# cmeraki/audiotoken

Measured on AMD Instinct MI355X. Metric: audio-sec tokenized / wall-sec (acoustic + semantic_m), higher is better.
Workload: dtype f32 (linear layers: two fp16 pieces per operand, three MFMA products, fp32 accumulate)

## Files before the change

audiotoken_amd/csrc/attention_f16x2_w8.hip:

```cpp
#include "at_common.h"
#include "w2vbert_kernels.h"
#include "split_scheme.h"

#include <cstdio>
#include <type_traits>

namespace at {

typedef __attribute__((address_space(3))) void w8_lds_void;

#ifdef W8_DEBUG_STAMPS
__device__ unsigned long long w8_stamps[2][12];
#define W8_T(i) const unsigned long long w8_t##i = __builtin_readcyclecounter()
#define W8_ACC(k, a_, b_) w8_d[k] += w8_t##b_ - w8_t##a_
#else
#define W8_T(i) do {} while (0)
#define W8_ACC(k, a_, b_) do {} while (0)
#endif

constexpr int W8_QB = 256, W8_KB = 64;
constexpr int W8_PLANE_B = W8_KB * 64 * 2;
constexpr int W8_TILE_B = 2 * W8_PLANE_B;
constexpr int W8_KBUFS = 2, W8_VBUFS = 2;
constexpr int W8_KV_B = (W8_KBUFS + W8_VBUFS) * W8_TILE_B;
constexpr int W8_QE_LD = 73;
constexpr int W8_LDS_MAX = 163840;
constexpr float W8_SCALE2 = 0.125f * 1.4426950408889634f;
constexpr float W8_P_LOG2 = 10.0f;
constexpr float W8_DEFER = 4.0f;
#ifndef W8_P_PIECES
#define W8_P_PIECES 2
#endif
constexpr int W8_PP = W8_P_PIECES;

static size_t w8_lds_bytes(int T, bool relpos) {
    const int nkt = (T + W8_KB - 1) / W8_KB;
    return (size_t)W8_KV_B + (relpos ? (size_t)W8_QB * W8_QE_LD * 4 : 0) + (size_t)nkt * W8_KB * 4 + 16;
}

__device__ __forceinline__ float w8_pair_max(float x) {
    const auto r = __builtin_amdgcn_permlane32_swap(__float_as_uint(x), __float_as_uint(x), false, false);
    return fmaxf(__uint_as_float(r[0]), __uint_as_float(r[1]));
}
__device__ __forceinline__ float w8_pair_sum(float x) {
    const auto r = __builtin_amdgcn_permlane32_swap(__float_as_uint(x), __float_as_uint(x), false, false);
    return __uint_as_float(r[0]) + __uint_as_float(r[1]);
}

__device__ __forceinline__ void w8_split_pair(float p0, float p1, unsigned& hi, unsigned& lo) {
    asm("v_cvt_pk_f16_f32 %0, %1, %2" : "=v"(hi) : "v"(p0), "v"(p1));
    asm("v_fma_mixlo_f16 %0, -%1, 1.0, %2 op_sel:[0,0,0] op_sel_hi:[1,0,0]" : "=v"(lo) : "v"(hi), "v"(p0));
    asm("v_fma_mixhi_f16 %0, -%1, 1.0, %2 op_sel:[1,0,0] op_sel_hi:[1,0,0]" : "+v"(lo) : "v"(hi), "v"(p1));
}

constexpr int W8_NQB = 1;
template <bool RELPOS>
__global__ __launch_bounds__(512 / W8_NQB, W8_NQB == 1 ? 2 : 1) void relpos_attention_w8_kernel(const float* __restrict__ qkv, const float* __restrict__ amask,
                                                                     const _Float16* __restrict__ dist_pieces, float dist_inv_scale, float* __restrict__ ctx, int T, int hid,
                                                                     int* __restrict__ status, _Float16* __restrict__ ctx_pieces, long long rows_pad,
                                                                     int nheads, int nclips, const _Float16* __restrict__ kv_pieces) {
    constexpr int NQB = W8_NQB;
    typedef SchemeF16x2 SC;
    typedef _Float16 PT;
    typedef f16x8 V8;
    typedef f16x4 V4;
    constexpr float XS = XB_F16_ACT_SCALE;
    constexpr float S_SCALE2 = W8_SCALE2 / (XS * XS);
    RangeMax over;
    extern __shared__ __attribute__((aligned(16))) unsigned char smem_raw[];
    const int nkt = (T + W8_KB - 1) / W8_KB;
    unsigned char* KV = smem_raw;
    float* QE = reinterpret_cast<float*>(KV + W8_KV_B);
    float* kbt = QE + (RELPOS ? W8_QB * W8_QE_LD : 0);
    int* tmask = reinterpret_cast<int*>(kbt + nkt * W8_KB);
    const int tid = threadIdx.x, lane = tid & 63;
    constexpr int NW = 8 / NQB, QW = 32 * NQB, NT = 64 * NW;
    const int wave = __builtin_amdgcn_readfirstlane(tid >> 6);
    const int l32 = lane & 31, hh = lane >> 5;
    const int nqt = (T + W8_QB - 1) / W8_QB;
    const int nblk = gridDim.x, per_xcd = (nblk + 7) >> 3;
    const int lid = (int)(blockIdx.x & 7) * per_xcd + (int)(blockIdx.x >> 3);
    if (lid >= nqt * nheads * nclips) return;
    const int qt = lid % nqt, pair = lid / nqt;
    const int h = pair % nheads, b = pair / nheads;
    const int l0 = qt * W8_QB;
    const long long rowbase = (long long)b * T;
    const int LD = 3 * hid;
    const float* qp = qkv + h * 64;

    const unsigned plane_b = (unsigned)(rows_pad * (long long)hid * 2);
    const __amdgpu_buffer_rsrc_t kvrs = __builtin_amdgcn_make_buffer_rsrc((void*)kv_pieces, 0, (int)(4u * plane_b), 0x00020000);
    constexpr int RW = 8 * NQB;
    const int d_row = wave * RW + (lane >> 3), d_cs = lane & 7;
    const unsigned clip_b = (unsigned)(rowbase * hid * 2 + h * 128);
    const int row_b = hid * 2;
    auto issue_k = [&](int kt, int buf) {
#pragma unroll
        for (int j = 0; j < NQB; ++j) {
            const int row = min(kt * W8_KB + d_row + 8 * j, T - 1);
            const unsigned vo = clip_b + (unsigned)(row * row_b) + ((d_cs ^ (((d_row + 8 * j) >> 1) & 7)) << 4);
#pragma unroll
            for (int p = 0; p < 2; ++p)
                __builtin_amdgcn_raw_ptr_buffer_load_lds(kvrs, (w8_lds_void*)(KV + buf * W8_TILE_B + wave * (RW * 128) + p * W8_PLANE_B + j * 1024), 16, vo, p * plane_b, 0, 0);
        }
    };
    auto issue_v = [&](int kt, int buf) {
#pragma unroll
        for (int j = 0; j < NQB; ++j) {
            const int row = min(kt * W8_KB + d_row + 8 * j, T - 1);
            const unsigned vo = clip_b + (unsigned)(row * row_b) + ((d_cs ^ ((((d_row + 8 * j) >> 1) & 1) << 2)) << 4);
#pragma unroll
            for (int p = 0; p < 2; ++p)
                __builtin_amdgcn_raw_ptr_buffer_load_lds(kvrs, (w8_lds_void*)(KV + (W8_KBUFS + buf) * W8_TILE_B + wave * (RW * 128) + p * W8_PLANE_B + j * 1024), 16, vo,
                                                         (2u + p) * plane_b, 0, 0);
        }
    };
    issue_k(0, 0);
    issue_v(0, 0);
    if (nkt > 1) issue_k(1, 1);

    const float FMIN = -3.4028234663852886e38f;
    if (tid < 2) tmask[tid] = 0;
    __syncthreads();
    for (int k = tid; k < nkt * W8_KB; k += NT) {
        float v = -INFINITY;
        if (k < T) v = amask[rowbase + k] != 0.f ? 0.f : FMIN;
        kbt[k] = v;
        if (v != 0.f) atomicOr(&tmask[k >> 11], 1 << ((k >> 6) & 31));
    }
    const int lq0 = l0 + wave * QW + l32;
    V8 qpc[NQB][2][4];
#pragma unroll
    for (int qb = 0; qb < NQB; ++qb) {
        const int lq = lq0 + 32 * qb;
        const int lc = lq < T ? lq : T - 1;
#pragma unroll
        for (int ds = 0; ds < 4; ++ds) {
            const f4 a = *reinterpret_cast<const f4*>(qp + (rowbase + lc) * LD + ds * 16 + 8 * hh);
            const f4 c = *reinterpret_cast<const f4*>(qp + (rowbase + lc) * LD + ds * 16 + 8 * hh + 4);
            V4 pa[2], pc[2];
            over |= split4<SC>(a, XS, pa);
            over |= split4<SC>(c, XS, pc);
#pragma unroll
            for (int i = 0; i < 2; ++i)
#pragma unroll
                for (int k = 0; k < 4; ++k) { qpc[qb][i][ds][k] = pa[i][k]; qpc[qb][i][ds][4 + k] = pc[i][k]; }
        }
    }
    if constexpr (RELPOS) {
        const float qe_scale = W8_SCALE2 * dist_inv_scale / XS;
#pragma unroll
        for (int qb = 0; qb < NQB; ++qb) {
            float* row = QE + (wave * QW + qb * 32 + l32) * W8_QE_LD;
#pragma unroll
            for (int rt = 0; rt < 3; ++rt) {
                f16v acc;
#pragma unroll
                for (int r = 0; r < 16; ++r) acc[r] = 0.f;
#pragma unroll
                for (int ds = 0; ds < 4; ++ds) {
                    V8 ef[2];
#pragma unroll
                    for (int p = 0; p < 2; ++p) ef[p] = *reinterpret_cast<const V8*>(dist_pieces + (p * 96 + rt * 32 + l32) * 64 + ds * 16 + 8 * hh);
#pragma unroll
                    for (int t = 0; t < SC::NPROD; ++t) acc = SC::mfma(ef[SC::prod_a(t)], qpc[qb][SC::prod_w(t)][ds], acc);
                }
#pragma unroll
                for (int r = 0; r < 16; ++r) {
                    const int bucket = rt * 32 + 8 * (r >> 2) + 4 * hh + (r & 3);
                    if (bucket < W8_QE_LD) row[bucket] = qe_scale * acc[r];
                }
            }
        }
    }
    f16v oacc[NQB][2];
#pragma unroll
    for (int qb = 0; qb < NQB; ++qb)
#pragma unroll
        for (int dt = 0; dt < 2; ++dt)
#pragma unroll
            for (int r = 0; r < 16; ++r) oacc[qb][dt][r] = 0.f;
    float mrun[NQB], lrun[NQB], alpha[NQB];
    bool rescale[NQB];
#pragma unroll
    for (int qb = 0; qb < NQB; ++qb) { mrun[qb] = -INFINITY; lrun[qb] = 0.f; alpha[qb] = 0.f; }
    const int wl_min = l0 + wave * QW, wl_max = wl_min + QW - 1;
    int koff[4];
#pragma unroll
    for (int ds = 0; ds < 4; ++ds) koff[ds] = l32 * 128 + (((2 * ds + hh) ^ ((l32 >> 1) & 7)) << 4);
    int voff[2];
    {
        const int li = lane & 15, vq = li >> 2, vp = li & 3;
        const int c0 = ((lane & 16) >> 3) + (vp >> 1), sv = (vq >> 1) & 1;
#pragma unroll
        for (int dt = 0; dt < 2; ++dt) voff[dt] = (4 * hh + vq) * 128 + ((((dt ^ sv) << 2) + c0) << 4) + (vp & 1) * 8;
    }
    asm volatile("s_waitcnt vmcnt(0)" ::: "memory");
    __syncthreads();
    const int tm0 = __builtin_amdgcn_readfirstlane(tmask[0]), tm1 = __builtin_amdgcn_readfirstlane(tmask[1]);
    typedef const __attribute__((address_space(3))) float lds_cf;
    typedef const __attribute__((address_space(3))) f4 lds_cf4;
    lds_cf* qe0 = (lds_cf*)(QE + (wave * QW + l32) * W8_QE_LD);
    lds_cf* kbt3 = (lds_cf*)kbt;
    float c_left[NQB], c_right[NQB];
#pragma unroll
    for (int qb = 0; qb < NQB; ++qb) { c_left[qb] = 0.f; c_right[qb] = 0.f; }
    if constexpr (RELPOS) {
#pragma unroll
        for (int qb = 0; qb < NQB; ++qb) { c_left[qb] = qe0[qb * 32 * W8_QE_LD]; c_right[qb] = qe0[qb * 32 * W8_QE_LD + 72]; }
    }

    auto s_tile = [&](f16v (&s)[NQB][2], int kbuf) {
        const unsigned char* Kb = KV + kbuf * W8_TILE_B;
#pragma unroll
        for (int kh = 0; kh < 2; ++kh) {
#pragma unroll
            for (int qb = 0; qb < NQB; ++qb)
#pragma unroll
                for (int r = 0; r < 16; ++r) s[qb][kh][r] = 0.f;
#pragma unroll
            for (int ds = 0; ds < 4; ++ds) {
                V8 kf[2];
#pragma unroll
                for (int p = 0; p < 2; ++p) kf[p] = *reinterpret_cast<const V8*>(Kb + p * W8_PLANE_B + kh * 32 * 128 + koff[ds]);
#pragma unroll
                for (int t = 0; t < SC::NPROD; ++t)
#pragma unroll
                    for (int qb = 0; qb < NQB; ++qb) s[qb][kh] = SC::mfma(kf[SC::prod_a(t)], qpc[qb][SC::prod_w(t)][ds], s[qb][kh]);
            }
        }
    };
    auto tile_fast = [&](int kt, bool& far_left) -> bool {
        const int r0 = kt * W8_KB;
        far_left = (r0 + W8_KB - 1) - wl_min <= -64;
        const bool far_right = r0 - wl_max >= 8;
        const bool masked = (((kt < 32 ? tm0 : tm1) >> (kt & 31)) & 1) != 0;
        return (!RELPOS || far_left || far_right) && !masked;
    };
    auto bias_pass = [&](f16v (&s)[2], int r0, int lq, lds_cf* qe, float c_far, auto near_) -> float {
        constexpr bool NEAR = decltype(near_)::value;
        float mx = -INFINITY;
#pragma unroll
        for (int kh = 0; kh < 2; ++kh)
#pragma unroll
            for (int g = 0; g < 4; ++g) {
                const int key0 = kh * 32 + 8 * g + 4 * hh;
                const f4 kb4 = *(lds_cf4*)(kbt3 + r0 + key0);
#pragma unroll
                for (int e = 0; e < 4; ++e) {
                    float bias = c_far;
                    if constexpr (NEAR) {
                        int dd = (r0 + key0 + e) - lq;
                        dd = dd < -64 ? -64 : (dd > 8 ? 8 : dd);
                        bias = qe[dd + 64];
                    }
                    const float sc = fmaf(S_SCALE2, s[kh][4 * g + e], bias + kb4[e]);
                    s[kh][4 * g + e] = sc;
                    mx = fmaxf(mx, sc);
                }
            }
        return mx;
    };
    auto softmax_general = [&](f16v (&s)[2], int kt, int qb) {
        const int r0 = kt * W8_KB;
        const int bmin = wl_min + 32 * qb, bmax = bmin + 31;
        const bool far_left = (r0 + W8_KB - 1) - bmin <= -64;
        const bool far_right = r0 - bmax >= 8;
        float mx;
        if (!RELPOS || far_left || far_right) mx = bias_pass(s, r0, 0, qe0, far_left ? c_left[qb] : c_right[qb], std::false_type{});
        else mx = bias_pass(s, r0, lq0 + 32 * qb, qe0 + qb * 32 * W8_QE_LD, 0.f, std::true_type{});
        mx = w8_pair_max(mx);
        const bool resc = __builtin_amdgcn_ballot_w64(mx > mrun[qb] + W8_DEFER) != 0ull;
        rescale[qb] = resc;
        const float mnew = resc ? fmaxf(mrun[qb], mx) : mrun[qb];
        const float sub = mnew - W8_P_LOG2;
        float rs = 0.f;
#pragma unroll
        for (int kh = 0; kh < 2; ++kh)
#pragma unroll
            for (int r = 0; r < 16; ++r) {
                const float p = __builtin_amdgcn_exp2f(s[kh][r] - sub);
                s[kh][r] = p;
                rs += p;
            }
        rs = w8_pair_sum(rs);
        alpha[qb] = resc ? __builtin_amdgcn_exp2f(mrun[qb] - mnew) : 1.0f;
        lrun[qb] = lrun[qb] * alpha[qb] + rs;
        mrun[qb] = mnew;
    };
    float f_mraw[NQB], f_mnew[NQB], f_bias2[NQB], f_rs[NQB], f_cfar[NQB];
    auto stat_slice = [&](f16v (&sa)[2], int qb, int k) {
        if (k < 4) {
            if (k == 0) { f_mraw[qb] = -INFINITY; f_rs[qb] = 0.f; }
#pragma unroll
            for (int e = 0; e < 8; ++e) f_mraw[qb] = fmaxf(f_mraw[qb], sa[k >> 1][8 * (k & 1) + e]);
        } else if (k == 4) {
            const float mx = w8_pair_max(fmaf(S_SCALE2, f_mraw[qb], f_cfar[qb]));
            const bool resc = __builtin_amdgcn_ballot_w64(mx > mrun[qb] + W8_DEFER) != 0ull;
            rescale[qb] = resc;
            f_mnew[qb] = resc ? fmaxf(mrun[qb], mx) : mrun[qb];
            f_bias2[qb] = (f_cfar[qb] - f_mnew[qb]) + W8_P_LOG2;
            alpha[qb] = resc ? __builtin_amdgcn_exp2f(mrun[qb] - f_mnew[qb]) : 1.0f;
        } else if (k < 21) {
#pragma unroll
            for (int e = 0; e < 2; ++e) {
                const int r = 2 * (k - 5) + e;
                const float p = __builtin_amdgcn_exp2f(fmaf(S_SCALE2, sa[r >> 4][r & 15], f_bias2[qb]));
                sa[r >> 4][r & 15] = p;
                f_rs[qb] += p;
            }
        } else if (k == 21) {
            const float rs = w8_pair_sum(f_rs[qb]);
            lrun[qb] = lrun[qb] * alpha[qb] + rs;
            mrun[qb] = f_mnew[qb];
        }
    };
    auto s_tile_softmax = [&](f16v (&sb)[NQB][2], int kbuf, f16v (&sa)[NQB][2]) {
        const unsigned char* Kb = KV + kbuf * W8_TILE_B;
        V8 kf[3][2];
        auto load_k = [&](int g) {
#pragma unroll
            for (int p = 0; p < 2; ++p) kf[g % 3][p] = *reinterpret_cast<const V8*>(Kb + p * W8_PLANE_B + (g >> 2) * 32 * 128 + koff[g & 3]);
        };
        load_k(0);
        load_k(1);
#pragma unroll
        for (int qb = 0; qb < NQB; ++qb)
#pragma unroll
            for (int kh = 0; kh < 2; ++kh)
#pragma unroll
                for (int r = 0; r < 16; ++r) sb[qb][kh][r] = 0.f;
        __builtin_amdgcn_sched_barrier(0);
#pragma unroll
        for (int g = 0; g < 8; ++g) {
            if (g + 2 < 8) load_k(g + 2);
#pragma unroll
            for (int t = 0; t < SC::NPROD; ++t)
#pragma unroll
                for (int qb = 0; qb < NQB; ++qb) {
                    sb[qb][g >> 2] = SC::mfma(kf[g % 3][SC::prod_a(t)], qpc[qb][SC::prod_w(t)][g & 3], sb[qb][g >> 2]);
                    const int sl = (3 * g + t) * NQB + qb;
                    if (sl < 22) stat_slice(sa[0], 0, sl);
                    else if (NQB > 1 && sl < 44) stat_slice(sa[NQB - 1], NQB - 1, sl - 22);
                    __builtin_amdgcn_sched_barrier(0);
                }
        }
    };
    auto pv_split = [&](const f16v (&s)[NQB][2], int vbuf) {
        const unsigned char* Vb = KV + (W8_KBUFS + vbuf) * W8_TILE_B;
        typedef short s4_ __attribute__((__vector_size__(4 * sizeof(short))));
        typedef unsigned u4_ __attribute__((ext_vector_type(4)));
        u4_ pp[2][NQB][2];
        auto split_pair = [&](int ks, int qb, int j) {
            unsigned hi, lo;
            if constexpr (W8_PP == 2) {
                w8_split_pair(s[qb][ks >> 1][8 * (ks & 1) + j], s[qb][ks >> 1][8 * (ks & 1) + j + 1], hi, lo);
                pp[ks & 1][qb][1][j >> 1] = lo;
            } else {
                asm("v_cvt_pk_f16_f32 %0, %1, %2" : "=v"(hi) : "v"(s[qb][ks >> 1][8 * (ks & 1) + j]), "v"(s[qb][ks >> 1][8 * (ks & 1) + j + 1]));
            }
            pp[ks & 1][qb][0][j >> 1] = hi;
        };
        V8 vf[2][2];
        auto load_v = [&](int u) {
#pragma unroll
            for (int p = 0; p < 2; ++p) {
                const unsigned char* vb = Vb + p * W8_PLANE_B + (u >> 1) * 16 * 128 + voff[u & 1];
                const s4_ lo = __builtin_amdgcn_ds_read_tr16_b64_v4i16((__attribute__((address_space(3))) s4_*)(vb));
                const s4_ hi = __builtin_amdgcn_ds_read_tr16_b64_v4i16((__attribute__((address_space(3))) s4_*)(vb + 8 * 128));
#pragma unroll
                for (int k = 0; k < 4; ++k) {
                    vf[u & 1][p][k] = __builtin_bit_cast(PT, (short)lo[k]);
                    vf[u & 1][p][4 + k] = __builtin_bit_cast(PT, (short)hi[k]);
                }
            }
        };
        load_v(0);
#pragma unroll
        for (int qb = 0; qb < NQB; ++qb)
#pragma unroll
            for (int j = 0; j < 8; j += 2) split_pair(0, qb, j);
        asm volatile("s_nop 1");
        __builtin_amdgcn_sched_barrier(0);
#pragma unroll
        for (int u = 0; u < 8; ++u) {
            const int ks = u >> 1, dt = u & 1;
            if (u + 1 < 8) load_v(u + 1);
            constexpr int T0 = W8_PP == 2 ? 0 : 1;
#pragma unroll
            for (int t = T0; t < SC::NPROD; ++t)
#pragma unroll
                for (int qb = 0; qb < NQB; ++qb) {
                    oacc[qb][dt] = SC::mfma(vf[u & 1][SC::prod_a(t)], __builtin_bit_cast(V8, pp[ks & 1][qb][SC::prod_w(t)]), oacc[qb][dt]);
                    const int sl = (dt * (SC::NPROD - T0) + (t - T0)) * NQB + qb;
                    if (ks + 1 < 4 && sl < 4 * NQB) split_pair(ks + 1, sl >> 2, 2 * (sl & 3));
                    __builtin_amdgcn_sched_barrier(0);
                }
        }
    };
#ifdef W8_DEBUG_STAMPS
    unsigned long long w8_d[8] = {0, 0, 0, 0, 0, 0, 0, 0};
    const unsigned long long w8_begin = __builtin_readcyclecounter();
#endif
    auto interval = [&](int i, f16v (&sa)[NQB][2], f16v (&sb)[NQB][2]) {
        W8_T(0);
        asm volatile("s_waitcnt vmcnt(0)" ::: "memory");
        W8_T(1);
        __builtin_amdgcn_s_barrier();
        W8_T(2);
        const bool more = i + 1 < nkt;
        if (i + 2 < nkt) issue_k(i + 2, i & 1);
        if (more) issue_v(i + 1, (i + 1) & 1);
        bool far_left;
        const bool fast = tile_fast(i, far_left);
        W8_T(3);
        if (more && fast) {
#pragma unroll
            for (int qb = 0; qb < NQB; ++qb) f_cfar[qb] = far_left ? c_left[qb] : c_right[qb];
            s_tile_softmax(sb, (i + 1) & 1, sa);
        } else {
            if (more) s_tile(sb, (i + 1) & 1);
            __builtin_amdgcn_sched_barrier(0);
            if (fast) {
#pragma unroll
                for (int qb = 0; qb < NQB; ++qb) {
                    f_cfar[qb] = far_left ? c_left[qb] : c_right[qb];
#pragma unroll
                    for (int k = 0; k < 22; ++k) stat_slice(sa[qb], qb, k);
                }
            } else {
#pragma unroll
                for (int qb = 0; qb < NQB; ++qb) softmax_general(sa[qb], i, qb);
            }
        }
        __builtin_amdgcn_sched_barrier(0);
        W8_T(4);
#pragma unroll
        for (int qb = 0; qb < NQB; ++qb)
            if (rescale[qb]) {
#pragma unroll
                for (int dt = 0; dt < 2; ++dt)
#pragma unroll
                    for (int r = 0; r < 16; ++r) oacc[qb][dt][r] *= alpha[qb];
            }
        __builtin_amdgcn_sched_barrier(0);
        W8_T(5);
        pv_split(sa, i & 1);
        W8_T(6);
#ifdef W8_DEBUG_STAMPS
        W8_ACC(0, 0, 1); W8_ACC(1, 1, 2); W8_ACC(2, 2, 3); W8_ACC(fast && more ? 3 : 4, 3, 4); W8_ACC(5, 4, 5); W8_ACC(6, 5, 6);
        w8_d[7] += (fast && more) ? 1 : 0;
#endif
    };
    f16v sA[NQB][2], sB[NQB][2];
    s_tile(sA, 0);
    for (int i = 0; i < nkt; i += 2) {
        interval(i, sA, sB);
        if (i + 1 < nkt) interval(i + 1, sB, sA);
    }
#ifdef W8_DEBUG_STAMPS
    if (blockIdx.x == (gridDim.x / 2) + 8 && (threadIdx.x == 0 || threadIdx.x == NT / 2)) {
        const int g = threadIdx.x ? 1 : 0;
        for (int k = 0; k < 8; ++k) w8_stamps[g][k] = w8_d[k];
        w8_stamps[g][8] = __builtin_readcyclecounter() - w8_begin;
        w8_stamps[g][9] = (unsigned long long)nkt;
    }
#endif
#pragma unroll
    for (int qb = 0; qb < NQB; ++qb) {
        const int lq = lq0 + 32 * qb;
        if (lq < T) {
            const float inv = (1.0f / lrun[qb]) * (1.0f / XS);
#pragma unroll
            for (int dt = 0; dt < 2; ++dt)
#pragma unroll
                for (int g = 0; g < 4; ++g) {
                    const f4 v = {oacc[qb][dt][4 * g] * inv, oacc[qb][dt][4 * g + 1] * inv, oacc[qb][dt][4 * g + 2] * inv, oacc[qb][dt][4 * g + 3] * inv};
                    if (ctx_pieces)
                        over |= store_pieces4<SC>(ctx_pieces, rows_pad * hid, rows_pad, rowbase + lq, h * 64 + dt * 32 + 8 * g + 4 * hh, v, XS);
                    else
                        *reinterpret_cast<f4*>(ctx + (rowbase + lq) * hid + h * 64 + dt * 32 + 8 * g + 4 * hh) = v;
                }
        }
    }
    range_publish(status, status ? status + 1 : nullptr, over);
}

bool relpos_attention_w8_eligible(int T, int heads, long long rows_pad, long long B, bool relpos) {
    return T >= 1 && T <= 4096  && rows_pad * heads * 64 * 8 < (1ll << 32)  && w8_lds_bytes(T, relpos) <= (size_t)W8_LDS_MAX && rows_pad >= B * T && (long long)T * heads * 64 * 2 < (1ll << 31);
}

int launch_relpos_attention_w8(const AttnArgs& a, hipStream_t stream) {
    const float *qkv = a.qkv, *amask = a.amask;
    float* const ctx = a.ctx;
    const int B = a.B, T = a.T, heads = a.heads;
    int* const status = a.status;
    __bf16* const ctx_pieces = a.ctx_pieces;
    const long long rows_pad = a.rows_pad;
    const __bf16 *kv_pieces = a.kv_pieces, *dist_pieces = a.dist.p;
    const float dist_scale = a.dist.s;
    AT_REQUIRE(kv_pieces != nullptr && relpos_attention_w8_eligible(T, heads, rows_pad, B, dist_pieces != nullptr),
               "relpos_attention_w8: needs pre-split k / v and a clip whose key-bias table fits LDS (T <= 1728 with rel-pos)");
    const long long nblk = (long long)((T + W8_QB - 1) / W8_QB) * heads * B;
    dim3 grid((unsigned)((nblk + 7) / 8 * 8));
    const size_t lds = w8_lds_bytes(T, dist_pieces != nullptr);
    const size_t lds_max = W8_LDS_MAX;
    int rc;
    const int hid = heads * 64;
    _Float16* cp = reinterpret_cast<_Float16*>(ctx_pieces);
    const _Float16* kp = reinterpret_cast<const _Float16*>(kv_pieces);
    const _Float16* dp = reinterpret_cast<const _Float16*>(dist_pieces);
    const float dinv = dist_pieces ? 1.0f / dist_scale : 1.0f;
    if (dist_pieces) {
        static LdsAttrFlags lds_attr;
        rc = set_max_dynamic_lds(lds_attr, relpos_attention_w8_kernel<true>, lds_max);
        if (!rc) hipLaunchKernelGGL((relpos_attention_w8_kernel<true>), grid, dim3(512 / W8_NQB), lds, stream, qkv, amask, dp, dinv, ctx, T, hid, status, cp, rows_pad, heads, B, kp);
    } else {
        static LdsAttrFlags lds_attr;
        rc = set_max_dynamic_lds(lds_attr, relpos_attention_w8_kernel<false>, lds_max);
        if (!rc) hipLaunchKernelGGL((relpos_attention_w8_kernel<false>), grid, dim3(512 / W8_NQB), lds, stream, qkv, amask, dp, dinv, ctx, T, hid, status, cp, rows_pad, heads, B, kp);
    }
    if (rc) return rc;
    AT_CHECK_HIP(hipGetLastError());
#ifdef W8_DEBUG_STAMPS
    {
        static int printed = 0;
        if (printed < 3) {
            ++printed;
            (void)hipStreamSynchronize(stream);
            unsigned long long hb[2][12];
            (void)hipMemcpyFromSymbol(hb, HIP_SYMBOL(w8_stamps), sizeof(hb));
            for (int g = 0; g < 2; ++g) {
                const double n = (double)(hb[g][9] ? hb[g][9] : 1), nf = (double)(hb[g][7] ? hb[g][7] : 1), ng = n - hb[g][7] > 0 ? n - hb[g][7] : 1;
                std::fprintf(stderr, "w8 stamps B %d T %d heads %d wave %d (cycles per 64-key interval, 64 queries): dma wait %.0f  barrier %.0f  issue+classify %.0f  phase A fast %.0f (x%llu)  phase A general/last %.0f (x%.0f)  rescale %.0f  phase B %.0f | loop total %.0f per interval, %llu intervals\n",
                             B, T, heads, g * 4, hb[g][0] / n, hb[g][1] / n, hb[g][2] / n, hb[g][3] / nf, hb[g][7], hb[g][4] / ng, ng, hb[g][5] / n, hb[g][6] / n, hb[g][8] / n, hb[g][9]);
            }
        }
    }
#endif
    return 0;
}

__global__ __launch_bounds__(256) void dist_split_kernel(const float* __restrict__ e, _Float16* __restrict__ out, float scale) {
    const int q = blockIdx.x * 256 + threadIdx.x;
    if (q >= 96 * 16) return;
    const int row = q >> 4, col = (q & 15) * 4;
    f4 v = {0.f, 0.f, 0.f, 0.f};
    if (row < 73) v = *reinterpret_cast<const f4*>(e + row * 64 + col);
    SchemeNoCheck<SchemeF16x2>::V4 p[2];
    split4<SchemeNoCheck<SchemeF16x2>>(v, scale, p);
#pragma unroll
    for (int i = 0; i < 2; ++i) *reinterpret_cast<f16x4*>(out + (i * 96 + row) * 64 + col) = p[i];
}
int launch_dist_split(const float* dist_emb, __bf16* out, float scale, hipStream_t stream) {
    hipLaunchKernelGGL(dist_split_kernel, dim3(6), dim3(256), 0, stream, dist_emb, reinterpret_cast<_Float16*>(out), scale);
    AT_CHECK_HIP(hipGetLastError());
    return 0;
}

__global__ __launch_bounds__(256) void kv_rowmajor_split_kernel(const float* __restrict__ qkv, _Float16* __restrict__ out, long long rows, long long rows_pad,
                                                                int hid, int* __restrict__ status) {
    typedef SchemeF16x2 SC;
    const long long q = (long long)blockIdx.x * 256 + threadIdx.x;
    const int qpr = hid / 4;
    RangeMax over;
    if (q < rows * 2 * qpr) {
        const long long row = q / (2 * qpr);
        const int rem = (int)(q - row * 2 * qpr), which = rem / qpr, col = (rem - which * qpr) * 4;
        const f4 v = *reinterpret_cast<const f4*>(qkv + row * 3 * hid + (1 + which) * hid + col);
        SC::V4 p[2];
        over |= split4<SC>(v, XB_F16_ACT_SCALE, p);
#pragma unroll
        for (int i = 0; i < 2; ++i) *reinterpret_cast<SC::V4*>(out + ((long long)(which * 2 + i) * rows_pad + row) * hid + col) = p[i];
    }
    range_publish(status, status ? status + 1 : nullptr, over);
}

int launch_kv_rowmajor_split(const float* qkv, __bf16* out, long long rows, long long rows_pad, int hid, int* status, hipStream_t stream) {
    AT_REQUIRE(hid % 4 == 0 && rows_pad >= rows, "kv_rowmajor_split: bad shape");
    const long long quads = rows * 2 * (hid / 4);
    hipLaunchKernelGGL(kv_rowmajor_split_kernel, dim3((unsigned)((quads + 255) / 256)), dim3(256), 0, stream, qkv, reinterpret_cast<_Float16*>(out), rows, rows_pad, hid,
                       status);
    AT_CHECK_HIP(hipGetLastError());
    return 0;
}

}
```

audiotoken_amd/csrc/dwconv_stream.hip:

```cpp
#include "at_common.h"
#include "w2vbert_kernels.h"
#include "split_scheme.h"

#include <type_traits>

namespace at {

namespace {

constexpr int DS_K = 31;
constexpr int DS_RB = 8;
constexpr int DS_WIN = DS_RB + DS_K - 1;
constexpr int DS_C = 1024;

__device__ __forceinline__ float ds_quad_xor1(float x) { return __builtin_bit_cast(float, __builtin_amdgcn_mov_dpp(__builtin_bit_cast(int, x), 0xB1, 0xF, 0xF, true)); }
__device__ __forceinline__ float ds_quad_xor2(float x) { return __builtin_bit_cast(float, __builtin_amdgcn_mov_dpp(__builtin_bit_cast(int, x), 0x4E, 0xF, 0xF, true)); }

template <bool SECOND>
__device__ __forceinline__ void ds_reduce(float (&v)[DS_RB], float (*sq)[256], float (*stat)[4], int c, int lane) {
#pragma unroll
    for (int i = 0; i < DS_RB; ++i) {
        float p = v[i] + ds_quad_xor1(v[i]);
        p = p + ds_quad_xor2(p);
        if ((lane & 3) == 0) sq[i][c >> 2] = p;
    }
    __syncthreads();
    const int wave = c >> 6;
    if (wave < DS_RB) {
        float t[4];
#pragma unroll
        for (int grp = 0; grp < 4; ++grp) t[grp] = sq[wave][grp * 64 + lane];
#pragma unroll
        for (int off = 32; off >= 1; off >>= 1)
#pragma unroll
            for (int grp = 0; grp < 4; ++grp) t[grp] += __shfl_xor(t[grp], off);
        if (lane == 0) {
            const float total = (t[0] + t[1]) + (t[2] + t[3]);
            if (!SECOND) {
                stat[wave][0] = total * (1.0f / 1024.0f);
            } else {
                const float vr = total * (1.0f / 1024.0f);
                const float rstd = 1.0f / sqrtf(vr + 1e-5f);
                stat[wave][1] = rstd;
                stat[wave][2] = -rstd * stat[wave][0];
            }
        }
    }
    __syncthreads();
}

}

template <class SC>
__global__ __launch_bounds__(1024, 1) void dwconv_stream_kernel(const float* __restrict__ g, const float* __restrict__ w ,
                                                                const float* __restrict__ gamma, const float* __restrict__ beta,
                                                                float* __restrict__ out, int T, int seg_len, void* __restrict__ pieces, long long rows_pad,
                                                                float scale, int* __restrict__ status) {
    __shared__ float sq[DS_RB][256];
    __shared__ __attribute__((aligned(16))) float stat[DS_RB][4];
    __shared__ __attribute__((aligned(16))) float otile[DS_RB][DS_C + 4];
    const int c = threadIdx.x, lane = c & 63;
    const int b = blockIdx.y;
    const int t_begin = blockIdx.x * seg_len;
    if (t_begin >= T) return;
    const int t_end = t_begin + seg_len < T ? t_begin + seg_len : T;
    const long long base = (long long)b * T;
    const float* gc = g + base * DS_C + c;

    float wt[DS_K];
#pragma unroll
    for (int j = 0; j < DS_K; ++j) wt[j] = w[j * DS_C + c];
    float xw[DS_WIN];
#pragma unroll
    for (int k = 0; k < DS_K - 1; ++k) {
        const int t = t_begin - (DS_K - 1) + k;
        xw[k] = t >= 0 ? gc[(long long)t * DS_C] : 0.f;
    }
    float pre[DS_RB];
    auto prefetch = [&](int tb) {
#pragma unroll
        for (int i = 0; i < DS_RB; ++i) {
            int t = tb + i;
            t = t < T ? t : T - 1;
            pre[i] = gc[(long long)t * DS_C];
        }
    };
    prefetch(t_begin);
    RangeMax over;
    (void)over;
    for (int tb = t_begin; tb < t_end; tb += DS_RB) {
#pragma unroll
        for (int i = 0; i < DS_RB; ++i) xw[DS_K - 1 + i] = pre[i];
        if (tb + DS_RB < t_end) prefetch(tb + DS_RB);
        float acc[DS_RB];
#pragma unroll
        for (int i = 0; i < DS_RB; ++i) {
            float a = 0.f;
#pragma unroll
            for (int tap = 0; tap < DS_K; ++tap) a = __builtin_fmaf(wt[tap], xw[i + tap], a);
            acc[i] = a;
        }
        float term[DS_RB];
#pragma unroll
        for (int i = 0; i < DS_RB; ++i) term[i] = acc[i];
        ds_reduce<false>(term, sq, stat, c, lane);
#pragma unroll
        for (int i = 0; i < DS_RB; ++i) {
            const float d = acc[i] - stat[i][0];
            const float m = __fmul_rn(d, d);
            const float f = __builtin_fmaf(d, d, ds_quad_xor1(m));
            term[i] = (lane & 1) ? 0.f : f;
        }
        ds_reduce<true>(term, sq, stat, c, lane);
        const float* gp = gamma;
        const float* bp = beta;
        asm volatile("" : "+s"(gp), "+s"(bp));
        const float gm = gp[c], bt = bp[c];
#pragma unroll
        for (int i = 0; i < DS_RB; ++i) {
            const int t = tb + i;
            const float o = swishf_(fmaf(fmaf(acc[i], stat[i][1], stat[i][2]), gm, bt));
            if constexpr (std::is_void<SC>::value) {
                if (t < t_end) out[(base + t) * DS_C + c] = o;
            } else {
                otile[i][c] = o;
            }
        }
        if constexpr (!std::is_void<SC>::value) {
            __syncthreads();
#pragma unroll
            for (int j = 0; j < 2; ++j) {
                const int e = c + 1024 * j, i = (e >> 2) & (DS_RB - 1), qd = ((e >> 5) << 2) | (e & 3);
                const int t = tb + i;
                if (t < t_end) {
                    const f4 o = *reinterpret_cast<const f4*>(&otile[i][qd * 4]);
                    over |= store_pieces4<SC>(reinterpret_cast<typename SC::T*>(pieces), rows_pad * DS_C, rows_pad, base + t, qd * 4, o, scale);
                }
            }
        }
#pragma unroll
        for (int k = 0; k < DS_K - 1; ++k) xw[k] = xw[k + DS_RB];
    }
    if constexpr (!std::is_void<SC>::value)
        if constexpr (SC::RANGE_CHECK)
            range_publish(status, status ? status + 1 : nullptr, over);
}

int launch_dwconv_stream(const float* g, const float* w, const float* gamma, const float* beta, float* out, int B, int T, hipStream_t stream,
                         const SplitOut& split) {
    __bf16* const pieces = split.pieces;
    const long long rows_pad = split.rows_pad;
    const int scheme = split.scheme;
    const float scale = split.scale;
    int* const status = split.status;
    const int cus = device_cus();
    int nseg = (cus + B - 1) / B;
    const int max_seg = (T + DS_RB - 1) / DS_RB;
    nseg = nseg < 1 ? 1 : (nseg > max_seg ? max_seg : nseg);
    const int seg_len = ((T + nseg - 1) / nseg + DS_RB - 1) / DS_RB * DS_RB;
    dim3 grid((T + seg_len - 1) / seg_len, B);
    if (pieces && scheme == XB_SCHEME_F16X2)
        hipLaunchKernelGGL((dwconv_stream_kernel<SchemeF16x2>), grid, dim3(1024), 0, stream, g, w, gamma, beta, out, T, seg_len, (void*)pieces, rows_pad, scale, status);
    else if (pieces)
        hipLaunchKernelGGL((dwconv_stream_kernel<SchemeBf16x3>), grid, dim3(1024), 0, stream, g, w, gamma, beta, out, T, seg_len, (void*)pieces, rows_pad, scale, status);
    else
        hipLaunchKernelGGL((dwconv_stream_kernel<void>), grid, dim3(1024), 0, stream, g, w, gamma, beta, out, T, seg_len, nullptr, 0LL, 1.0f, nullptr);
    AT_CHECK_HIP(hipGetLastError());
    return 0;
}

}
```

Measured before the change: 15720.

## Overlap next dwconv window FMAs with LayerNorm reduction barriers

Software-pipelines the depthwise-conv stream kernel so that the next 8-row window's convolution FMAs (split in two halves) are computed between the two barriers of each LayerNorm statistic reduction, hiding barrier waits. It also rewrites the cross-wave reduction to use 16 lanes with vector LDS reads and DPP row rotations instead of a 64-lane shuffle tree, and forces v_fmac via inline asm. Separately it adds debug cycle-stamp instrumentation (compiled out by default) to the attention and dwconv kernels. The pipelining raises register pressure by keeping a second accumulator array live.

```diff
diff --git a/audiotoken_amd/csrc/attention_f16x2_w8.hip b/audiotoken_amd/csrc/attention_f16x2_w8.hip
--- a/audiotoken_amd/csrc/attention_f16x2_w8.hip
+++ b/audiotoken_amd/csrc/attention_f16x2_w8.hip
@@ -10,11 +10,13 @@
 typedef __attribute__((address_space(3))) void w8_lds_void;
 
 #ifdef W8_DEBUG_STAMPS
-__device__ unsigned long long w8_stamps[2][12];
+__device__ unsigned long long w8_stamps[2][32];
+#define W8_P(i) __builtin_amdgcn_sched_barrier(0); const unsigned long long w8_p##i = __builtin_readcyclecounter(); __builtin_amdgcn_sched_barrier(0)
 #define W8_T(i) const unsigned long long w8_t##i = __builtin_readcyclecounter()
 #define W8_ACC(k, a_, b_) w8_d[k] += w8_t##b_ - w8_t##a_
 #else
 #define W8_T(i) do {} while (0)
+#define W8_P(i) do {} while (0)
 #define W8_ACC(k, a_, b_) do {} while (0)
 #endif
 
@@ -67,6 +69,9 @@
     constexpr float XS = XB_F16_ACT_SCALE;
     constexpr float S_SCALE2 = W8_SCALE2 / (XS * XS);
     RangeMax over;
+#ifdef W8_DEBUG_STAMPS
+    const unsigned long long w8_entry = __builtin_readcyclecounter();
+#endif
     extern __shared__ __attribute__((aligned(16))) unsigned char smem_raw[];
     const int nkt = (T + W8_KB - 1) / W8_KB;
     unsigned char* KV = smem_raw;
@@ -120,14 +125,17 @@
     if (nkt > 1) issue_k(1, 1);
 
     const float FMIN = -3.4028234663852886e38f;
+    W8_P(1);
     if (tid < 2) tmask[tid] = 0;
     __syncthreads();
+    W8_P(2);
     for (int k = tid; k < nkt * W8_KB; k += NT) {
         float v = -INFINITY;
         if (k < T) v = amask[rowbase + k] != 0.f ? 0.f : FMIN;
         kbt[k] = v;
         if (v != 0.f) atomicOr(&tmask[k >> 11], 1 << ((k >> 6) & 31));
     }
+    W8_P(3);
     const int lq0 = l0 + wave * QW + l32;
     V8 qpc[NQB][2][4];
 #pragma unroll
@@ -147,6 +155,7 @@
                 for (int k = 0; k < 4; ++k) { qpc[qb][i][ds][k] = pa[i][k]; qpc[qb][i][ds][4 + k] = pc[i][k]; }
         }
     }
+    W8_P(4);
     if constexpr (RELPOS) {
         const float qe_scale = W8_SCALE2 * dist_inv_scale / XS;
 #pragma unroll
@@ -173,6 +182,7 @@
             }
         }
     }
+    W8_P(5);
     f16v oacc[NQB][2];
 #pragma unroll
     for (int qb = 0; qb < NQB; ++qb)
@@ -195,8 +205,11 @@
 #pragma unroll
         for (int dt = 0; dt < 2; ++dt) voff[dt] = (4 * hh + vq) * 128 + ((((dt ^ sv) << 2) + c0) << 4) + (vp & 1) * 8;
     }
+    W8_P(6);
     asm volatile("s_waitcnt vmcnt(0)" ::: "memory");
+    W8_P(7);
     __syncthreads();
+    W8_P(8);
     const int tm0 = __builtin_amdgcn_readfirstlane(tmask[0]), tm1 = __builtin_amdgcn_readfirstlane(tmask[1]);
     typedef const __attribute__((address_space(3))) float lds_cf;
     typedef const __attribute__((address_space(3))) f4 lds_cf4;
@@ -400,6 +413,8 @@
     };
 #ifdef W8_DEBUG_STAMPS
     unsigned long long w8_d[8] = {0, 0, 0, 0, 0, 0, 0, 0};
+    unsigned long long w8_c[3] = {0, 0, 0}, w8_n[3] = {0, 0, 0}, w8_prev = 0, w8_first = 0;
+    int w8_cls = 0;
     const unsigned long long w8_begin = __builtin_readcyclecounter();
 #endif
     auto interval = [&](int i, f16v (&sa)[NQB][2], f16v (&sb)[NQB][2]) {
@@ -408,6 +423,20 @@
         W8_T(1);
         __builtin_amdgcn_s_barrier();
         W8_T(2);
+#ifdef W8_DEBUG_STAMPS
+        {
+            if (i > 0) w8_c[w8_cls] += w8_t2 - w8_prev; else w8_first = w8_t2 - w8_begin;
+            w8_prev = w8_t2;
+            const bool masked_i = (((i < 32 ? tm0 : tm1) >> (i & 31)) & 1) != 0;
+            bool all_fast = !masked_i;
+            for (int w = 0; w < NW; ++w) {
+                const int a = l0 + w * QW, b2 = a + QW - 1;
+                if (RELPOS && !((i * W8_KB + W8_KB - 1) - a <= -64) && !(i * W8_KB - b2 >= 8)) all_fast = false;
+            }
+            w8_cls = i == nkt - 1 ? 2 : (all_fast ? 0 : 1);
+            ++w8_n[w8_cls];
+        }
+#endif
         const bool more = i + 1 < nkt;
         if (i + 2 < nkt) issue_k(i + 2, i & 1);
         if (more) issue_v(i + 1, (i + 1) & 1);
@@ -459,12 +488,8 @@
         if (i + 1 < nkt) interval(i + 1, sB, sA);
     }
 #ifdef W8_DEBUG_STAMPS
-    if (blockIdx.x == (gridDim.x / 2) + 8 && (threadIdx.x == 0 || threadIdx.x == NT / 2)) {
-        const int g = threadIdx.x ? 1 : 0;
-        for (int k = 0; k < 8; ++k) w8_stamps[g][k] = w8_d[k];
-        w8_stamps[g][8] = __builtin_readcyclecounter() - w8_begin;
-        w8_stamps[g][9] = (unsigned long long)nkt;
-    }
+    const unsigned long long w8_loop_end = __builtin_readcyclecounter();
+    w8_c[w8_cls] += w8_loop_end - w8_prev;
 #endif
 #pragma unroll
     for (int qb = 0; qb < NQB; ++qb) {
@@ -484,6 +509,24 @@
         }
     }
     range_publish(status, status ? status + 1 : nullptr, over);
+#ifdef W8_DEBUG_STAMPS
+    asm volatile("s_waitcnt vmcnt(0)" ::: "memory");
+    if (blockIdx.x == (gridDim.x / 2) + 8 && (threadIdx.x == 0 || threadIdx.x == NT / 2)) {
+        const unsigned long long w8_exit = __builtin_readcyclecounter();
+        const int g = threadIdx.x ? 1 : 0;
+        for (int k = 0; k < 8; ++k) w8_stamps[g][k] = w8_d[k];
+        w8_stamps[g][8] = w8_loop_end - w8_begin;
+        w8_stamps[g][9] = (unsigned long long)nkt;
+        w8_stamps[g][10] = w8_begin - w8_entry;
+        w8_stamps[g][11] = w8_first;
+        for (int k = 0; k < 3; ++k) { w8_stamps[g][12 + 2 * k] = w8_c[k]; w8_stamps[g][13 + 2 * k] = w8_n[k]; }
+        w8_stamps[g][18] = w8_exit - w8_loop_end;
+        w8_stamps[g][19] = w8_exit - w8_entry;
+        w8_stamps[g][20] = w8_p1 - w8_entry; w8_stamps[g][21] = w8_p2 - w8_p1; w8_stamps[g][22] = w8_p3 - w8_p2; w8_stamps[g][23] = w8_p4 - w8_p3;
+        w8_stamps[g][24] = w8_p5 - w8_p4; w8_stamps[g][25] = w8_p6 - w8_p5; w8_stamps[g][26] = w8_p7 - w8_p6; w8_stamps[g][27] = w8_p8 - w8_p7;
+        w8_stamps[g][28] = w8_begin - w8_p8;
+    }
+#endif
 }
 
 bool relpos_attention_w8_eligible(int T, int heads, long long rows_pad, long long B, bool relpos) {
@@ -525,15 +568,23 @@
 #ifdef W8_DEBUG_STAMPS
     {
         static int printed = 0;
+        static long long shape = 0;
+        if (shape != (long long)B * 65536 + T) { shape = (long long)B * 65536 + T; printed = 0; }
         if (printed < 3) {
             ++printed;
             (void)hipStreamSynchronize(stream);
-            unsigned long long hb[2][12];
+            unsigned long long hb[2][32];
             (void)hipMemcpyFromSymbol(hb, HIP_SYMBOL(w8_stamps), sizeof(hb));
             for (int g = 0; g < 2; ++g) {
                 const double n = (double)(hb[g][9] ? hb[g][9] : 1), nf = (double)(hb[g][7] ? hb[g][7] : 1), ng = n - hb[g][7] > 0 ? n - hb[g][7] : 1;
                 std::fprintf(stderr, "w8 stamps B %d T %d heads %d wave %d (cycles per 64-key interval, 64 queries): dma wait %.0f  barrier %.0f  issue+classify %.0f  phase A fast %.0f (x%llu)  phase A general/last %.0f (x%.0f)  rescale %.0f  phase B %.0f | loop total %.0f per interval, %llu intervals\n",
                              B, T, heads, g * 4, hb[g][0] / n, hb[g][1] / n, hb[g][2] / n, hb[g][3] / nf, hb[g][7], hb[g][4] / ng, ng, hb[g][5] / n, hb[g][6] / n, hb[g][8] / n, hb[g][9]);
+                const double life = (double)(hb[g][19] ? hb[g][19] : 1);
+                std::fprintf(stderr, "w8 lifetime B %d T %d heads %d wave %d (cycles): prologue %llu  first S + wait %llu  all-fast intervals %llu (x%llu)  some-wave-general intervals %llu (x%llu)  last interval %llu (x%llu)  epilogue %llu  lifetime %llu | outside the loop %.2f %%\n",
+                             B, T, heads, g * 4, hb[g][10], hb[g][11], hb[g][12], hb[g][13], hb[g][14], hb[g][15], hb[g][16], hb[g][17], hb[g][18], hb[g][19],
+                             100.0 * (double)(hb[g][10] + hb[g][11] + hb[g][18]) / life);
+                std::fprintf(stderr, "w8 prologue B %d T %d heads %d wave %d (cycles): arguments + load issue %llu  first barrier %llu  key-bias table %llu  q split %llu  rel-pos table %llu  accumulators + offsets %llu  wait K/V DMA %llu  barrier %llu  far-field constants %llu\n",
+                             B, T, heads, g * 4, hb[g][20], hb[g][21], hb[g][22], hb[g][23], hb[g][24], hb[g][25], hb[g][26], hb[g][27], hb[g][28]);
             }
         }
     }
diff --git a/audiotoken_amd/csrc/dwconv_stream.hip b/audiotoken_amd/csrc/dwconv_stream.hip
--- a/audiotoken_amd/csrc/dwconv_stream.hip
+++ b/audiotoken_amd/csrc/dwconv_stream.hip
@@ -2,6 +2,7 @@
 #include "w2vbert_kernels.h"
 #include "split_scheme.h"
 
+#include <cstdio>
 #include <type_traits>
 
 namespace at {
@@ -12,30 +13,68 @@
 constexpr int DS_RB = 8;
 constexpr int DS_WIN = DS_RB + DS_K - 1;
 constexpr int DS_C = 1024;
+typedef std::integral_constant<int, 0> DS_LO;
+typedef std::integral_constant<int, DS_RB / 2> DS_HI;
+
+#ifdef DS_DEBUG_STAMPS
+__device__ unsigned long long ds_stamps[2][12];
+#define DS_STAMP_PARAMS , unsigned long long (&ds_d)[12], unsigned long long& ds_last
+#define DS_STAMP_ARGS , ds_d, ds_last
+#define DS_T(k)                                                    \
+    do {                                                           \
+        __builtin_amdgcn_sched_barrier(0);                         \
+        const unsigned long long t_ = __builtin_readcyclecounter(); \
+        ds_d[k] += t_ - ds_last;                                   \
+        ds_last = t_;                                              \
+        __builtin_amdgcn_sched_barrier(0);                         \
+    } while (0)
+#else
+#define DS_STAMP_PARAMS
+#define DS_STAMP_ARGS
+#define DS_T(k) do {} while (0)
+#endif
+
+__device__ __forceinline__ float ds_fma(float w, float x, float a) {
+    asm("v_fmac_f32 %0, %1, %2" : "+v"(a) : "v"(w), "v"(x));
+    return a;
+}
 
 __device__ __forceinline__ float ds_quad_xor1(float x) { return __builtin_bit_cast(float, __builtin_amdgcn_mov_dpp(__builtin_bit_cast(int, x), 0xB1, 0xF, 0xF, true)); }
 __device__ __forceinline__ float ds_quad_xor2(float x) { return __builtin_bit_cast(float, __builtin_amdgcn_mov_dpp(__builtin_bit_cast(int, x), 0x4E, 0xF, 0xF, true)); }
 
-template <bool SECOND>
-__device__ __forceinline__ void ds_reduce(float (&v)[DS_RB], float (*sq)[256], float (*stat)[4], int c, int lane) {
+__device__ __forceinline__ float ds_row_ror8(float x) { return __builtin_bit_cast(float, __builtin_amdgcn_mov_dpp(__builtin_bit_cast(int, x), 0x128, 0xF, 0xF, true)); }
+__device__ __forceinline__ float ds_row_ror4(float x) { return __builtin_bit_cast(float, __builtin_amdgcn_mov_dpp(__builtin_bit_cast(int, x), 0x124, 0xF, 0xF, true)); }
+
+template <bool SECOND, class F>
+__device__ __forceinline__ void ds_reduce(float (&v)[DS_RB], float (*sq)[256], float (*stat)[4], int c, int lane, F&& overlap DS_STAMP_PARAMS) {
+    const int slot = (((c >> 6) & 3) * 16 + ((((c >> 8) & 1) << 1) | (c >> 9)) * 4 + ((lane >> 2) & 3)) * 4 + (lane >> 4);
 #pragma unroll
     for (int i = 0; i < DS_RB; ++i) {
         float p = v[i] + ds_quad_xor1(v[i]);
         p = p + ds_quad_xor2(p);
-        if ((lane & 3) == 0) sq[i][c >> 2] = p;
-    }
+        if ((lane & 3) == 0) sq[i][slot] = p;
+    }
+    DS_T(1);
+    __builtin_amdgcn_sched_barrier(0);
     __syncthreads();
+    __builtin_amdgcn_sched_barrier(0);
+    DS_T(2);
     const int wave = c >> 6;
-    if (wave < DS_RB) {
-        float t[4];
-#pragma unroll
-        for (int grp = 0; grp < 4; ++grp) t[grp] = sq[wave][grp * 64 + lane];
-#pragma unroll
-        for (int off = 32; off >= 1; off >>= 1)
-#pragma unroll
-            for (int grp = 0; grp < 4; ++grp) t[grp] += __shfl_xor(t[grp], off);
+    if (wave < DS_RB && lane < 16) {
+        f4 a[4];
+#pragma unroll
+        for (int m = 0; m < 4; ++m) a[m] = *reinterpret_cast<const f4*>(&sq[wave][(m * 16 + lane) * 4]);
+        float b[4], e[2];
+#pragma unroll
+        for (int n = 0; n < 4; ++n) b[n] = (a[0][n] + a[2][n]) + (a[1][n] + a[3][n]);
+        e[0] = b[0] + b[2];
+        e[1] = b[1] + b[3];
+        float t = e[0] + e[1];
+        t = t + ds_quad_xor2(t);
+        t = t + ds_quad_xor1(t);
+        t = t + ds_row_ror8(t);
+        const float total = t + ds_row_ror4(t);
         if (lane == 0) {
-            const float total = (t[0] + t[1]) + (t[2] + t[3]);
             if (!SECOND) {
                 stat[wave][0] = total * (1.0f / 1024.0f);
             } else {
@@ -46,7 +85,13 @@
             }
         }
     }
+    DS_T(3);
+    overlap();
+    DS_T(9);
+    __builtin_amdgcn_sched_barrier(0);
     __syncthreads();
+    __builtin_amdgcn_sched_barrier(0);
+    DS_T(4);
 }
 
 }
@@ -56,7 +101,7 @@
                                                                 const float* __restrict__ gamma, const float* __restrict__ beta,
                                                                 float* __restrict__ out, int T, int seg_len, void* __restrict__ pieces, long long rows_pad,
                                                                 float scale, int* __restrict__ status) {
-    __shared__ float sq[DS_RB][256];
+    __shared__ __attribute__((aligned(16))) float sq[DS_RB][256];
     __shared__ __attribute__((aligned(16))) float stat[DS_RB][4];
     __shared__ __attribute__((aligned(16))) float otile[DS_RB][DS_C + 4];
     const int c = threadIdx.x, lane = c & 63;
@@ -88,22 +133,47 @@
     prefetch(t_begin);
     RangeMax over;
     (void)over;
+#ifdef DS_DEBUG_STAMPS
+    unsigned long long ds_d[12] = {0, 0, 0, 0, 0, 0, 0, 0, 0, 0, 0, 0};
+    const unsigned long long ds_begin = __builtin_readcyclecounter();
+    unsigned long long ds_last = ds_begin;
+#endif
+    auto next_window = [&](int tb_after) {
+#pragma unroll
+        for (int i = 0; i < DS_RB; ++i) xw[DS_K - 1 + i] = pre[i];
+        if (tb_after < t_end) prefetch(tb_after);
+    };
+    auto fma_half = [&](float (&a_)[DS_RB], auto lo_) {
+        constexpr int LO = decltype(lo_)::value;
+#pragma unroll
+        for (int i = LO; i < LO + DS_RB / 2; ++i) {
+            float a = 0.f;
+#pragma unroll
+            for (int tap = 0; tap < DS_K; ++tap) a = ds_fma(wt[tap], xw[i + tap], a);
+            a_[i] = a;
+        }
+    };
+    float acc[DS_RB];
+    next_window(t_begin + DS_RB);
+    fma_half(acc, DS_LO{});
+    fma_half(acc, DS_HI{});
+    DS_T(0);
     for (int tb = t_begin; tb < t_end; tb += DS_RB) {
-#pragma unroll
-        for (int i = 0; i < DS_RB; ++i) xw[DS_K - 1 + i] = pre[i];
-        if (tb + DS_RB < t_end) prefetch(tb + DS_RB);
-        float acc[DS_RB];
-#pragma unroll
-        for (int i = 0; i < DS_RB; ++i) {
-            float a = 0.f;
-#pragma unroll
-            for (int tap = 0; tap < DS_K; ++tap) a = __builtin_fmaf(wt[tap], xw[i + tap], a);
-            acc[i] = a;
-        }
+        const bool more = tb + DS_RB < t_end;
+        float accn[DS_RB];
+#pragma unroll
+        for (int i = 0; i < DS_RB; ++i) accn[i] = 0.f;
         float term[DS_RB];
 #pragma unroll
         for (int i = 0; i < DS_RB; ++i) term[i] = acc[i];
-        ds_reduce<false>(term, sq, stat, c, lane);
+        ds_reduce<false>(term, sq, stat, c, lane, [&] {
+            if (more) {
+#pragma unroll
+                for (int k = 0; k < DS_K - 1; ++k) xw[k] = xw[k + DS_RB];
+                next_window(tb + 2 * DS_RB);
+                fma_half(accn, DS_LO{});
+            }
+        } DS_STAMP_ARGS);
 #pragma unroll
         for (int i = 0; i < DS_RB; ++i) {
             const float d = acc[i] - stat[i][0];
@@ -111,7 +181,10 @@
             const float f = __builtin_fmaf(d, d, ds_quad_xor1(m));
             term[i] = (lane & 1) ? 0.f : f;
         }
-        ds_reduce<true>(term, sq, stat, c, lane);
+        DS_T(5);
+        ds_reduce<true>(term, sq, stat, c, lane, [&] {
+            if (more) fma_half(accn, DS_HI{});
+        } DS_STAMP_ARGS);
         const float* gp = gamma;
         const float* bp = beta;
         asm volatile("" : "+s"(gp), "+s"(bp));
@@ -126,8 +199,10 @@
                 otile[i][c] = o;
             }
         }
+        DS_T(6);
         if constexpr (!std::is_void<SC>::value) {
             __syncthreads();
+            DS_T(7);
 #pragma unroll
             for (int j = 0; j < 2; ++j) {
                 const int e = c + 1024 * j, i = (e >> 2) & (DS_RB - 1), qd = ((e >> 5) << 2) | (e & 3);
@@ -138,9 +213,19 @@
                 }
             }
         }
-#pragma unroll
-        for (int k = 0; k < DS_K - 1; ++k) xw[k] = xw[k + DS_RB];
-    }
+        DS_T(8);
+#pragma unroll
+        for (int i = 0; i < DS_RB; ++i) acc[i] = accn[i];
+#ifdef DS_DEBUG_STAMPS
+        ++ds_d[10];
+#endif
+    }
+#ifdef DS_DEBUG_STAMPS
+    if (blockIdx.x == gridDim.x / 2 && blockIdx.y == gridDim.y / 2 && (c == 0 || c == DS_C - 64)) {
+        ds_d[11] = __builtin_readcyclecounter() - ds_begin;
+        for (int k = 0; k < 12; ++k) ds_stamps[c ? 1 : 0][k] = ds_d[k];
+    }
+#endif
     if constexpr (!std::is_void<SC>::value)
         if constexpr (SC::RANGE_CHECK)
             range_publish(status, status ? status + 1 : nullptr, over);
@@ -166,6 +251,27 @@
     else
         hipLaunchKernelGGL((dwconv_stream_kernel<void>), grid, dim3(1024), 0, stream, g, w, gamma, beta, out, T, seg_len, nullptr, 0LL, 1.0f, nullptr);
     AT_CHECK_HIP(hipGetLastError());
+#ifdef DS_DEBUG_STAMPS
+    {
+        static int printed = 0;
+        static long long shape = 0;
+        if (shape != (long long)B * 65536 + T) { shape = (long long)B * 65536 + T; printed = 0; }
+        if (printed < 2) {
+            ++printed;
+            (void)hipStreamSynchronize(stream);
+            unsigned long long hb[2][12];
+            (void)hipMemcpyFromSymbol(hb, HIP_SYMBOL(ds_stamps), sizeof(hb));
+            static const char* const names[10] = {"first window + FMA", "quad sums + hand-off", "wait hand-off barrier", "tree + statistic", "wait publishing barrier",
+                                                  "squared deviations", "normalise + swish", "wait tile barrier", "piece stores", "next window + FMA"};
+            for (int g = 0; g < 2; ++g) {
+                const double n = (double)(hb[g][10] ? hb[g][10] : 1), tot = (double)(hb[g][11] ? hb[g][11] : 1);
+                std::fprintf(stderr, "dwconv stamps B %d T %d pieces %d wave %d: %llu iterations, %.0f cycles each |", B, T, pieces ? 1 : 0, g * 15, hb[g][10], tot / n);
+                for (int k = 0; k < 10; ++k) std::fprintf(stderr, " %s %.0f (%.1f %%) |", names[k], hb[g][k] / n, 100.0 * hb[g][k] / tot);
+                std::fprintf(stderr, " barrier + tree wait %.1f %%\n", 100.0 * (double)(hb[g][2] + hb[g][3] + hb[g][4] + hb[g][7]) / tot);
+            }
+        }
+    }
+#endif
     return 0;
 }
 
```

Result: no change. 15760 (median of 6 runs) (+0.3%).
